# rrahn/libspm

Measured on AMD Instinct MI355X. Metric: Gbases/s scanned, Myers k<=3 |P|=100, higher is better.
Workload: dtype u32

## Files before the change

libspm_amd/csrc/filter.hpp:

```cpp
#pragma once

#include "brute.hpp"
#include "common.hpp"
#include "filter_shared.hpp"
#include "pack.hpp"
#include "hd.hpp"

namespace spm_hip
{

struct survivor
{
    uint32_t key;
    uint32_t t_lo, t_hi;
    uint32_t pad;
};
constexpr uint32_t kSurvInvalid = 0xFFFFFFFFu;

struct band_rec
{
    uint32_t slot;
    uint32_t val;
    uint32_t seg;
    uint32_t band;
// ... 295 lines not shown
            const bool act = todo != 0;
            const uint32_t b = act ? (uint32_t)__ffs(todo) - 1u : 0u;
            todo &= todo - 1;
            const uint32_t u = b & 1u, d = (b >> 1) + 1u;
            const uint32_t wu = (j + 1 < NWD && u) ? w[j + 1 < NWD ? j + 1 : j] : w[j];
            const uint32_t pu = (j + 1 < NWD && u) ? prev[j + 1 < NWD ? j + 1 : j] : prev[j];
            const uint32_t key = (uint32_t)((((uint64_t)wu << 32) | pu) >> (2 * d));
            const uint32_t x = chd_hash(key).x;
            const uint32_t dsp = disp_tab[x >> P.chd_bucket_shift];
            const uint32_t slot = ((x >> 3) + dsp * ((key | 1u) & 0xFFFFFFu)) & P.chd_slot_mask;
            const uint32_t f = fp_tab[slot];
            const bool hit = act && ((f ^ key ^ (key >> 16)) & 0xFFFFu) == 0;
            if (__ballot(hit) != 0) {
                if (__builtin_amdgcn_readfirstlane(cand_chunk_of(P, lds)[5]) != 0)
                    return;
                const uint64_t wpos = gbase + (uint64_t)(j + u) * 1024 + (uint64_t)lane * 16;
                const int64_t ts = (int64_t)wpos - 16 + (int64_t)d;
                const bool has = hit && ts >= (int64_t)P.lo && (uint64_t)ts + P.key_len <= P.hi;
                emit_survivors(P, has, key, has ? (uint64_t)ts : 0, lane, lds);
            }
        }
    }
}

template <int S, int UU, int HV, int SIG, bool KM, bool AN = false>
__device__ __forceinline__ void filter_group(const filter_params &P, const uint4 (&cur)[UU], uint64_t gbase,
                                             uint32_t &carry_in, uint32_t &carry_n, uint32_t lane,
                                             const uint32_t *lds, uint32_t idx_mask)
{
    uint32_t w[UU], prev[UU];
    uint32_t nv[SIG != 4 ? UU : 1];
#pragma unroll
    for (int u = 0; u < UU; ++u) {
        uint32_t nm = 0;
        w[u] = pack16_sig<SIG>(cur[u], nm);
        prev[u] = __builtin_amdgcn_update_dpp(0u, w[u], 0x138 , 0xF, 0xF, false);
        if (lane == 0)
            prev[u] = carry_in;
        carry_in = __builtin_amdgcn_readlane(w[u], 63);
        if (SIG != 4) {
            uint32_t np = __builtin_amdgcn_update_dpp(0u, nm, 0x138, 0xF, 0xF, false);
            if (lane == 0)
                np = carry_n;
            carry_n = __builtin_amdgcn_readlane(nm, 63);
            nv[u] = (nm << 16) | np;
        }
    }
    if constexpr (AN)
        filter_words_anchored<UU>(P, w, prev, gbase, lane, lds);
    else
        filter_words<S, UU, HV, SIG, false, KM>(P, w, prev, nv, gbase, lane, lds, idx_mask);
}

template <int S, int U, int HV, int SIG, bool KM, bool AN = false>
__global__ __launch_bounds__(((S == 1 && !KM && SIG == 4) || (S == 2 && U == 2)) ? 1024 : 512) void seed_filter_kernel(const filter_params P)
{
    extern __shared__ uint32_t lds[];
    for (uint32_t i = threadIdx.x; i < P.lds_words; i += blockDim.x)
        lds[i] = P.bitmap[i];
    if ((threadIdx.x & 63) == 0) {
        uint32_t *ck = lds + P.lds_words + kCandLdsSlot + kCandRec * (threadIdx.x >> 6);
        for (uint32_t i = 0; i < kCandRec; ++i)
            ck[i] = 0;
    }
    __syncthreads();

    const uint32_t lane = threadIdx.x & 63;
    const uint32_t waves_per_wg = blockDim.x >> 6;
    const uint64_t wave_id =
        (uint64_t)blockIdx.x * waves_per_wg + (uint32_t)__builtin_amdgcn_readfirstlane(threadIdx.x >> 6);
    const uint64_t n_waves = (uint64_t)gridDim.x * waves_per_wg;
    const uint32_t idx_mask = P.bitmap_words * 32 - 1;

    const uint64_t base0 = P.lo & ~1023ull;
    const uint64_t n_chunks = (P.hi - base0 + 1023) / 1024;
    const uint64_t n_whole = (P.hi - base0) / 1024;
    const uint64_t span = P.span_chunks;
    const uint64_t n_spans = (n_chunks + span - 1) / span;
    const uint8_t *lane_text = P.text + base0 + (uint64_t)lane * 16;

    const uint32_t wave_in_wg = (uint32_t)__builtin_amdgcn_readfirstlane(threadIdx.x >> 6);
    uint64_t sp = wave_id;
    for (;;) {
        if (P.dynamic == 1) {
            unsigned long long t = 0;
            if (lane == 0)
                t = atomicAdd(&P.counters[kCntSpanHead], 1ull);
            sp = ((unsigned long long)__builtin_amdgcn_readfirstlane((uint32_t)(t >> 32)) << 32) |
                 (uint32_t)__builtin_amdgcn_readfirstlane((uint32_t)t);
        } else if (P.dynamic == 2) {
            __syncthreads();
            if (threadIdx.x == 0) {
                const unsigned long long t = atomicAdd(&P.counters[kCntSpanHead], (unsigned long long)waves_per_wg);
                lds[P.lds_words] = (uint32_t)t;
                lds[P.lds_words + 1] = (uint32_t)(t >> 32);
            }
            __syncthreads();
            const uint64_t base = ((uint64_t)(uint32_t)__builtin_amdgcn_readfirstlane(lds[P.lds_words + 1]) << 32) |
                                  (uint32_t)__builtin_amdgcn_readfirstlane(lds[P.lds_words]);
            if (base >= n_spans)
                break;
            sp = base + wave_in_wg;
            if (sp >= n_spans)
                continue;
        }
        if (sp >= n_spans)
            break;
        const uint64_t c_begin = sp * span;
        const uint64_t c_end = c_begin + span < n_chunks ? c_begin + span : n_chunks;
        span_open(P, lds, lane, base0 + c_begin * 1024);
        uint32_t carry_in = 0, carry_n = 0;
        {
            const uint64_t cb = base0 + c_begin * 1024;
            if (cb >= 16 && lane == 0) {
                const uint4 before = load_text16(P.text, cb - 16, P.hi);
                carry_in = pack16_sig<SIG>(before, carry_n);
            }
            carry_in = __builtin_amdgcn_readfirstlane(carry_in);
            carry_n = __builtin_amdgcn_readfirstlane(carry_n);
        }
        uint64_t ch = c_begin;
        const uint64_t whole_end = c_end < n_whole ? c_end : n_whole;
        const uint64_t fast_end = c_begin + (whole_end > c_begin ? (whole_end - c_begin) / U * U : 0);
        if (ch < fast_end) {
            uint4 nxt[U];
#pragma unroll
            for (int u = 0; u < U; ++u)
                nxt[u] = load16_stream(lane_text + (ch + u) * 1024);
            for (; ch < fast_end; ch += U) {
                uint4 cur[U];
#pragma unroll
                for (int u = 0; u < U; ++u)
                    cur[u] = nxt[u];
                const bool more = ch + U < fast_end;
                const uint64_t pf = more ? ch + U : ch;
                const uint64_t ustride = more ? 1024 : 0;
#pragma unroll
                for (int u = 0; u < U; ++u)
                    nxt[u] = load16_stream(lane_text + pf * 1024 + (uint64_t)u * ustride);
                if constexpr (S <= 2)
                    __builtin_amdgcn_sched_barrier(0);
                filter_group<S, U, HV, SIG, KM, AN>(P, cur, base0 + ch * 1024, carry_in, carry_n, lane, lds, idx_mask);
            }
        }
        for (; ch < c_end; ++ch) {
            uint4 one[1];
            one[0] = load_text16(P.text, base0 + ch * 1024 + (uint64_t)lane * 16, P.hi);
            filter_group<S, 1, HV, SIG, KM, AN>(P, one, base0 + ch * 1024, carry_in, carry_n, lane, lds, idx_mask);
        }
        sp += n_waves;
    }
    surv_close(P, cand_chunk_of(P, lds), lane);
}

constexpr uint32_t kDenseQueueCap = 192;
constexpr int kDenseBatches = 3;

template <int NP>
__device__ __forceinline__ uint32_t dense_select(const filter_params &P, uint32_t w, uint32_t prev)
{
    const uint32_t X = alignbit(w, prev, 2);
    const uint32_t Y = alignbit(w, prev, 4);
    uint32_t sel = 0;
#pragma unroll
    for (int i = 0; i < NP; ++i) {
        const uint32_t C0 = (P.pat_c[i] & 3u) * 0x55555555u, M0 = (P.pat_cm[i] & 3u) * 0x55555555u;
        const uint32_t C1 = (P.pat_c[i] >> 2) * 0x55555555u, M1 = (P.pat_cm[i] >> 2) * 0x55555555u;
        uint32_t t = ((X ^ C0) & M0) | ((Y ^ C1) & M1);
        t |= t >> 1;
        sel |= ~t;
    }
    return sel & 0x55555555u;
}

struct dense_queue
{
    uint32_t key[kDenseQueueCap];
    uint32_t off[kDenseQueueCap];
};

__device__ __forceinline__ void dense_drain(const filter_params &P, dense_queue &Q, uint32_t &qn, bool all, uint64_t span_base,
                                            uint32_t lane, const uint32_t *lds)
{
    while (qn >= 64 || (all && qn != 0)) {
        const uint32_t nb_full = qn >> 6;
        uint32_t nb = all ? (qn + 63) >> 6 : nb_full;
        nb = nb > (uint32_t)kDenseBatches ? (uint32_t)kDenseBatches : nb;
        uint32_t key[kDenseBatches], off[kDenseBatches];
        uint4 bk[kDenseBatches];
        bool v[kDenseBatches];
#pragma unroll
        for (int b = 0; b < kDenseBatches; ++b) {
            const int32_t e = (int32_t)qn - 64 * b - 1 - (int32_t)lane;
            v[b] = (uint32_t)b < nb && e >= 0;
            key[b] = 0;
            off[b] = 0;
            bk[b] = make_uint4(0, 0, 0, 0);
            if (v[b]) {
                key[b] = Q.key[e];
                off[b] = Q.off[e];
                bk[b] = P.buckets[dense_bucket(key[b], P.bucket_shift)];
            }
        }
// ... 42 lines not shown
        uint32_t pm = 0;
        if constexpr (S == 0) {
            uint32_t todo = dense_select<NP>(P, w0, p0);
            if (pair)
                todo |= dense_select<NP>(P, w1, p1) << 1;
            while (todo != 0) {
                const uint32_t b = (uint32_t)__ffs(todo) - 1u;
                todo &= todo - 1;
                const bool odd = (b & 1u) != 0;
                const uint64_t both = ((uint64_t)(odd ? w1 : w0) << 32) | (odd ? p1 : p0);
                const uint32_t key = (uint32_t)(both >> ((b & ~1u) + 2u));
                const uint32_t h = key ^ (key >> 13);
                const uint32_t word = *reinterpret_cast<const uint32_t *>(reinterpret_cast<const uint8_t *>(lds) + ((h >> 3) & 0x1FFFCu));
                pm |= __builtin_amdgcn_ubfe(word, h, 1) << b;
            }
        } else {
#pragma unroll
            for (int u = 0; u < (pair ? 2 : 1); ++u) {
#pragma unroll
                for (int d = S; d <= 16; d += S) {
                    const uint32_t wu = u ? w1 : w0, pu = u ? p1 : p0;
                    const uint32_t key = (d == 16 ? wu : alignbit(wu, pu, (2 * d) & 31)) & kmask;
                    const uint32_t h = key ^ (key >> 13);
                    const uint32_t word = *reinterpret_cast<const uint32_t *>(reinterpret_cast<const uint8_t *>(lds) + ((h >> 3) & 0x1FFFCu));
                    pm |= __builtin_amdgcn_ubfe(word, h, 1) << (2 * (d - 1) + u);
                }
            }
        }
        while (__ballot(pm != 0) != 0) {
            const bool pos = pm != 0;
            const uint32_t b = pos ? (uint32_t)__ffs(pm) - 1u : 0u;
            pm &= pm - 1;
            const bool odd = (b & 1u) != 0;
            const uint64_t both = ((uint64_t)(odd ? w1 : w0) << 32) | (odd ? p1 : p0);
            const uint32_t key = (uint32_t)(both >> ((b & ~1u) + 2u)) & kmask;
            const uint64_t mm = __ballot(pos);
            if (pos) {
                const uint32_t q = qn + __popcll(mm & ((1ull << lane) - 1));
                Q.key[q] = key;
                Q.off[q] = goff + (uint32_t)j * 1024u + (odd ? 1024u : 0u) + (b >> 1) + 1u;
            }
            qn += __popcll(mm);
            __builtin_amdgcn_fence(__ATOMIC_RELEASE, "wavefront");
            __builtin_amdgcn_wave_barrier();
            if (qn > kDenseQueueCap - 64)
                dense_drain(P, Q, qn, false, span_base, lane, lds);
        }
    }
}

template <int U, int NP, int S = 0, bool KM = false>
__global__ __launch_bounds__(1024) void seed_filter_dense_kernel(const filter_params P)
{
    extern __shared__ uint32_t lds[];
    for (uint32_t i = threadIdx.x; i < P.lds_words; i += blockDim.x)
        lds[i] = P.bitmap[i];
    if ((threadIdx.x & 63) == 0) {
        uint32_t *ck = lds + P.lds_words + kCandLdsSlot + kCandRec * (threadIdx.x >> 6);
        for (uint32_t i = 0; i < kCandRec; ++i)
            ck[i] = 0;
    }
    __syncthreads();

    const uint32_t lane = threadIdx.x & 63;
    const uint32_t waves_per_wg = blockDim.x >> 6;
    const uint32_t wave_in_wg = (uint32_t)__builtin_amdgcn_readfirstlane(threadIdx.x >> 6);
    const uint64_t wave_id = (uint64_t)blockIdx.x * waves_per_wg + wave_in_wg;
    const uint64_t n_waves = (uint64_t)gridDim.x * waves_per_wg;
    dense_queue &Q = *reinterpret_cast<dense_queue *>(lds + P.lds_words + kCandLdsSlot + kCandRec * 16 +
                                                      (sizeof(dense_queue) / 4) * wave_in_wg);
    uint32_t qn = 0;

    const uint64_t base0 = P.lo & ~1023ull;
    const uint64_t n_chunks = (P.hi - base0 + 1023) / 1024;
    const uint64_t n_whole = (P.hi - base0) / 1024;
    const uint64_t span = P.span_chunks;
    const uint64_t n_spans = (n_chunks + span - 1) / span;
    const uint8_t *lane_text = P.text + base0 + (uint64_t)lane * 16;

    uint64_t sp = wave_id;
    for (;;) {
        if (P.dynamic == 1) {
            unsigned long long t = 0;
            if (lane == 0)
                t = atomicAdd(&P.counters[kCntSpanHead], 1ull);
            sp = ((unsigned long long)__builtin_amdgcn_readfirstlane((uint32_t)(t >> 32)) << 32) |
                 (uint32_t)__builtin_amdgcn_readfirstlane((uint32_t)t);
        } else if (P.dynamic == 2) {
            __syncthreads();
            if (threadIdx.x == 0) {
                const unsigned long long t = atomicAdd(&P.counters[kCntSpanHead], (unsigned long long)waves_per_wg);
                lds[P.lds_words] = (uint32_t)t;
                lds[P.lds_words + 1] = (uint32_t)(t >> 32);
            }
            __syncthreads();
            const uint64_t base = ((uint64_t)(uint32_t)__builtin_amdgcn_readfirstlane(lds[P.lds_words + 1]) << 32) |
                                  (uint32_t)__builtin_amdgcn_readfirstlane(lds[P.lds_words]);
            if (base >= n_spans)
                break;
            sp = base + wave_in_wg;
            if (sp >= n_spans)
                continue;
        }
        if (sp >= n_spans)
            break;
        const uint64_t c_begin = sp * span;
        const uint64_t c_end = c_begin + span < n_chunks ? c_begin + span : n_chunks;
        const uint64_t span_base = base0 + c_begin * 1024;
        span_open(P, lds, lane, span_base);
        uint32_t carry_in = 0;
        {
            uint32_t nm = 0;
            if (span_base >= 16 && lane == 0)
                carry_in = pack16_sig<4>(load_text16(P.text, span_base - 16, P.hi), nm);
            carry_in = __builtin_amdgcn_readfirstlane(carry_in);
        }
        uint64_t ch = c_begin;
        const uint64_t whole_end = c_end < n_whole ? c_end : n_whole;
        const uint64_t fast_end = c_begin + (whole_end > c_begin ? (whole_end - c_begin) / U * U : 0);
        if (ch < fast_end) {
            uint4 nxt[U];
#pragma unroll
            for (int u = 0; u < U; ++u)
                nxt[u] = load16_stream(lane_text + (ch + u) * 1024);
            for (; ch < fast_end; ch += U) {
                uint4 cur[U];
#pragma unroll
                for (int u = 0; u < U; ++u)
                    cur[u] = nxt[u];
                const bool more = ch + U < fast_end;
                const uint64_t pf = more ? ch + U : ch;
                const uint64_t ustride = more ? 1024 : 0;
#pragma unroll
                for (int u = 0; u < U; ++u)
                    nxt[u] = load16_stream(lane_text + pf * 1024 + (uint64_t)u * ustride);
                __builtin_amdgcn_sched_barrier(0);
                dense_group<U, NP, S, KM>(P, cur, base0 + ch * 1024, span_base, carry_in, lane, lds, Q, qn);
            }
        }
        for (; ch < c_end; ++ch) {
            uint4 one[1];
            one[0] = load_text16(P.text, base0 + ch * 1024 + (uint64_t)lane * 16, P.hi);
            dense_group<1, NP, S, KM>(P, one, base0 + ch * 1024, span_base, carry_in, lane, lds, Q, qn);
        }
        dense_drain(P, Q, qn, true, span_base, lane, lds);
        sp += n_waves;
    }
    surv_close(P, cand_chunk_of(P, lds), lane);
}

template <int S, int U2, int HV, bool KM>
__global__ __launch_bounds__(1024) void seed_filter_packed_kernel(const filter_params P, const uint4 *__restrict__ shadow)
{
    extern __shared__ uint32_t lds[];
    for (uint32_t i = threadIdx.x; i < P.lds_words; i += blockDim.x)
        lds[i] = P.bitmap[i];
    if ((threadIdx.x & 63) == 0) {
        uint32_t *ck = lds + P.lds_words + kCandLdsSlot + kCandRec * (threadIdx.x >> 6);
        for (uint32_t i = 0; i < kCandRec; ++i)
            ck[i] = 0;
    }
    __syncthreads();

    constexpr int NWD = 4 * U2;
    const uint32_t lane = threadIdx.x & 63;
    const uint32_t waves_per_wg = blockDim.x >> 6;
    const uint32_t wave_in_wg = (uint32_t)__builtin_amdgcn_readfirstlane(threadIdx.x >> 6);
    const uint64_t wave_id = (uint64_t)blockIdx.x * waves_per_wg + wave_in_wg;
    const uint64_t n_waves = (uint64_t)gridDim.x * waves_per_wg;
    const uint32_t idx_mask = P.bitmap_words * 32 - 1;

    const uint64_t base0 = P.lo & ~4095ull;
    const uint64_t n_chunks = (P.hi - base0 + 4095) / 4096;
    const uint64_t span = P.span_chunks;
    const uint64_t n_spans = (n_chunks + span - 1) / span;
    const uint4 *lane_src = shadow + (base0 / 64) + lane;

    uint64_t sp = wave_id;
    for (;;) {
        if (P.dynamic == 1) {
            unsigned long long t = 0;
            if (lane == 0)
                t = atomicAdd(&P.counters[kCntSpanHead], 1ull);
            sp = ((unsigned long long)__builtin_amdgcn_readfirstlane((uint32_t)(t >> 32)) << 32) |
                 (uint32_t)__builtin_amdgcn_readfirstlane((uint32_t)t);
        } else if (P.dynamic == 2) {
            __syncthreads();
            if (threadIdx.x == 0) {
                const unsigned long long t = atomicAdd(&P.counters[kCntSpanHead], (unsigned long long)waves_per_wg);
                lds[P.lds_words] = (uint32_t)t;
                lds[P.lds_words + 1] = (uint32_t)(t >> 32);
            }
            __syncthreads();
            const uint64_t base = ((uint64_t)(uint32_t)__builtin_amdgcn_readfirstlane(lds[P.lds_words + 1]) << 32) |
                                  (uint32_t)__builtin_amdgcn_readfirstlane(lds[P.lds_words]);
            if (base >= n_spans)
                break;
            sp = base + wave_in_wg;
            if (sp >= n_spans)
                continue;
        }
        if (sp >= n_spans)
            break;
        const uint64_t c_begin = sp * span;
        const uint64_t c_end = c_begin + span < n_chunks ? c_begin + span : n_chunks;
        const uint64_t fast_end = c_begin + (c_end - c_begin + U2 - 1) / U2 * U2;
        span_open(P, lds, lane, base0 + c_begin * 4096);
        uint32_t carry_in = 0;
        {
            const uint64_t first_word = (base0 + c_begin * 4096) / 16;
            if (first_word > 0 && lane == 0)
                carry_in = reinterpret_cast<const uint32_t *>(shadow)[first_word - 1];
            carry_in = __builtin_amdgcn_readfirstlane(carry_in);
        }
        uint4 nxt[U2];
#pragma unroll
        for (int u = 0; u < U2; ++u)
            nxt[u] = load16_stream(reinterpret_cast<const uint8_t *>(lane_src + (c_begin + u) * 64));
        for (uint64_t ch = c_begin; ch < fast_end; ch += U2) {
            uint4 cur[U2];
#pragma unroll
            for (int u = 0; u < U2; ++u)
                cur[u] = nxt[u];
            const bool more = ch + U2 < fast_end;
            const uint64_t pf = more ? ch + U2 : ch;
            const uint64_t ustride = more ? 64 : 0;
#pragma unroll
            for (int u = 0; u < U2; ++u)
                nxt[u] = load16_stream(reinterpret_cast<const uint8_t *>(lane_src + pf * 64 + (uint64_t)u * ustride));
            __builtin_amdgcn_sched_barrier(0);
            uint32_t w[NWD], prev[NWD];
            const uint32_t nv[1] = {0};
#pragma unroll
            for (int u = 0; u < U2; ++u) {
                w[4 * u + 0] = cur[u].x;
                w[4 * u + 1] = cur[u].y;
                w[4 * u + 2] = cur[u].z;
                w[4 * u + 3] = cur[u].w;
                uint32_t p0 = __builtin_amdgcn_update_dpp(0u, cur[u].w, 0x138 , 0xF, 0xF, false);
                if (lane == 0)
                    p0 = carry_in;
                carry_in = __builtin_amdgcn_readlane(cur[u].w, 63);
                prev[4 * u + 0] = p0;
                prev[4 * u + 1] = cur[u].x;
                prev[4 * u + 2] = cur[u].y;
                prev[4 * u + 3] = cur[u].z;
            }
            filter_words<S, NWD, HV, 4, true, KM>(P, w, prev, nv, base0 + ch * 4096, lane, lds, idx_mask);
        }
        sp += n_waves;
    }
    surv_close(P, cand_chunk_of(P, lds), lane);
}

struct verify_params
{
    const uint8_t *text;
    uint64_t text_alloc;
    uint64_t ctx_begin;
    uint64_t scan_begin;
    uint64_t scan_end;
    uint64_t pos_offset;
    const band_rec *bands;
    const unsigned long long *counters;
    uint32_t band_counter;
    uint32_t preselected;
    uint64_t band_cap;
    ulonglong2 *band_tab;
    uint32_t table_mask, band_bits;
    uint32_t runs;
    const uint8_t *surplus;
    uint32_t Bw;
    uint32_t overlap;
    uint32_t max_m;
    const uint32_t *peq32;
    uint32_t sigma;
    uint32_t nw_table;
    uint32_t max_k;
    const int32_t *m;
    const int32_t *k;
    uint32_t report_begin;
    uint32_t max_span;
    uint32_t wave_text;
    unsigned long long *seen;
    uint32_t seen_mask;
    spm_hit *hits;
    unsigned long long *hit_counter;
    uint64_t hit_cap;
    unsigned long long *overflow;
    const uint64_t *seg_offsets;
    uint64_t n_segments;
    const uint32_t *seg_owned;
};

struct resolve_params
{
    const survivor *surv;
    unsigned long long *counters;
    uint64_t surv_cap;
    const pass_entry *passes;
    const uint4 *entries;
    uint32_t key_len;
    uint32_t flank_check;
// ... 1254 lines not shown
```

libspm_amd/csrc/internal.hpp:

```cpp
#pragma once

#include <algorithm>
#include <chrono>
#include <cmath>
#include <cstdlib>
#include <cstring>
#include <memory>

#include "common.hpp"
#include "index_build.hpp"

using namespace spm_hip;

struct spm_patterns : spm_hip::seed_index
{
    spm_ctx *ctx = nullptr;
    int algo = 0;
    uint32_t n = 0;
    uint32_t sigma = 4;
    std::vector<uint8_t> ranks;
    std::vector<uint32_t> offsets;
    std::vector<int32_t> m, k;
    uint32_t n_groups = 0;
    uint32_t max_m = 0;
    uint32_t max_window = 0;
    uint32_t max_k = 0;
    uint32_t NW = 1;
    bool is_myers() const { return algo == SPM_ALGO_MYERS || algo == SPM_ALGO_MYERS_PREFIX; }
    void *d_arena = nullptr;
    uint32_t *d_peq = nullptr;
    uint32_t *d_peq_bot = nullptr;
    uint32_t *d_peq_verify = nullptr;
    uint32_t *d_hp0 = nullptr;
    int32_t *d_m = nullptr;
    int32_t *d_k = nullptr;
    mutable uint64_t cand_hint = 0;
    uint8_t *d_surplus = nullptr;
    uint8_t *d_ranks = nullptr;
    uint32_t *d_offsets = nullptr;
    uint32_t *d_needle_pk = nullptr;
    uint32_t *d_pk_offsets = nullptr;
    uint16_t *d_seed_q = nullptr;
    pass_entry *d_pass_tab = nullptr;
    uint4 *d_entries = nullptr;
    mutable uint64_t hit_hint = 0;
    mutable bool scanned = false;
    mutable int exact_whole = -1;
    mutable uint64_t band_hint = 0;
    spm_build_stats build{};
    mutable void *d_align = nullptr;
    mutable const uint64_t *d_al_rpeq = nullptr;
    mutable const uint32_t *d_al_rpeq_off = nullptr;
    mutable const uint8_t *d_al_ranks = nullptr;
    mutable const uint32_t *d_al_offsets = nullptr;
};

using clk = std::chrono::steady_clock;
inline float ms_since(clk::time_point t) { return std::chrono::duration<float, std::milli>(clk::now() - t).count(); }
inline bool spm_trace_on()
{
    const char *v = getenv("SPM_HIP_TRACE");
    return v && *v && *v != '0';
}


struct scan_tuning
{
    int cand_cap = 0;
    int brute_cutoff = 1;
    int verify_wave_min_words = 8;
    int span_budget = 0;
    int verify_runs = 1;
    int verify_runs_min_bands = 65536;
    int band_cap = 0;
    static scan_tuning from_env()
    {
        scan_tuning T;
        T.cand_cap = env_int("SPM_HIP_FILTER_CAND_CAP", 0);
        T.brute_cutoff = env_int("SPM_HIP_BRUTE_CUTOFF", 1);
        T.verify_wave_min_words = env_int("SPM_HIP_VERIFY_WAVE_MIN_WORDS", 8);
        T.span_budget = env_int("SPM_HIP_FILTER_SPAN_BUDGET", 0);
        T.verify_runs = env_int("SPM_HIP_VERIFY_RUNS", 1);
        T.verify_runs_min_bands = env_int("SPM_HIP_VERIFY_RUNS_MIN_BANDS", 65536);
        T.band_cap = env_int("SPM_HIP_FILTER_BAND_CAP", 0);
        return T;
    }
};

struct scan_args
{
    spm_ctx *ctx;
    const spm_text *text;
    uint64_t begin, end, ctx_begin;
    const spm_patterns *ps;
    spm_scan_opts opts;
    spm_hits *hits;
    scan_tuning tune;
    const uint64_t *seg_offsets = nullptr;
    uint64_t n_segments = 0;
    const uint64_t *d_seg_offsets = nullptr;
    const uint32_t *d_seg_owned = nullptr;
};

struct scan_state
{
    retry_state retry;
    filter_result filt;
    const uint64_t *segs = nullptr;
    std::vector<uint64_t> seg_host;
    const std::vector<uint64_t> *tiles = nullptr;
};

void state_to_internal(const spm_patterns *p, const void *state, std::vector<uint32_t> &out);
void state_from_internal(const spm_patterns *p, const std::vector<uint32_t> &in, void *state);
int text_alloc(spm_ctx *ctx, uint64_t n, uint32_t sigma, spm_text **out);
int ensure_scratch(spm_ctx *ctx, size_t bytes);
int run_brute(const scan_args &A, const scan_state &S, uint64_t begin, uint64_t end, uint64_t ctx_begin,
              const uint32_t *d_state_in, uint32_t *d_state_out, bool report, bool single_tile);
int run_filter(const scan_args &A, const retry_state &R, filter_result &out);
int scan_impl(spm_ctx *ctx, const spm_text *text, uint64_t begin, uint64_t end, const spm_patterns *patterns,
              const spm_scan_opts *opts_in, const void *state_in, void *state_out, const uint64_t *seg_offsets,
              uint64_t n_segments, spm_hits **out, const uint64_t *d_seg_offsets = nullptr,
              const uint32_t *d_seg_owned = nullptr, const std::function<int(spm_hits *)> *after_launch = nullptr);

struct align_work
{
    const spm_patterns *ps = nullptr;
    const spm_text *text = nullptr;
    uint64_t pos_offset = 0;
    const spm_hit *hits = nullptr;
    uint64_t n = 0;
    const uint64_t *lo = nullptr;
    const uint32_t *cig_off = nullptr;
    bool begin_only = false;
// ... 18 lines not shown
```

libspm_amd/csrc/scan_filter.hip:

```cpp
#include "internal.hpp"
#include "filter.hpp"

namespace
{
template <typename K, typename... Args>
void launch(K kernel, dim3 grid, uint32_t threads, size_t lds, hipStream_t s, Args... args)
{
    hipFuncSetAttribute((const void *)kernel, hipFuncAttributeMaxDynamicSharedMemorySize, (int)lds);
    hipLaunchKernelGGL(kernel, grid, dim3(threads), lds, s, args...);
}

using filter_kernel = void (*)(filter_params);
using packed_kernel = void (*)(filter_params, const uint4 *);

template <int S, int U, bool KM>
filter_kernel sparse_kernel(uint32_t hv, uint32_t sigma)
{
    if (hv == 2 && sigma == 5)
        return seed_filter_kernel<S, U, 2, 5, KM>;
    if (hv == 2 && sigma == 15)
        return seed_filter_kernel<S, U, 2, 15, KM>;
    if (hv == 1 && sigma == 4)
        return seed_filter_kernel<S, U, 1, 4, KM>;
    if constexpr (S >= 4)
// ... 19 lines not shown
        if (F.stride == 2)
            return km ? seed_filter_dense_kernel<4, 1, 2, true> : seed_filter_dense_kernel<4, 1, 2, false>;
        return nullptr;
    }
    switch (F.stride) {
    case 16: return km ? nullptr : sparse_kernel<16, 8, false>(F.hash_variant, sigma);
    case 8: return km ? nullptr : sparse_kernel<8, 8, false>(F.hash_variant, sigma);
    case 4: return km ? nullptr : sparse_kernel<4, 8, false>(F.hash_variant, sigma);
    case 2: return km ? sparse_kernel<2, 2, true>(F.hash_variant, sigma) : sparse_kernel<2, 2, false>(F.hash_variant, sigma);
    case 1:
        if (F.anchor_cm != 0 && F.hash_variant == 2 && sigma == 4 && !km)
            return seed_filter_kernel<1, 4, 2, 4, false, true>;
        return km ? sparse_kernel<1, 2, true>(F.hash_variant, sigma) : sparse_kernel<1, 2, false>(F.hash_variant, sigma);
    default: return nullptr;
    }
}

packed_kernel select_packed_kernel(uint32_t stride, bool km)
{
    if (km)
        return nullptr;
    switch (stride) {
    case 16: return seed_filter_packed_kernel<16, 4, 2, false>;
    case 8: return seed_filter_packed_kernel<8, 4, 2, false>;
    case 4: return seed_filter_packed_kernel<4, 2, 2, false>;
    default: return nullptr;
    }
}

template <int NWN>
void launch_verify_nw(const verify_params &V, dim3 grid, hipStream_t s)
{
    uint32_t threads = 256;
    const size_t per_thread = (size_t)(V.sigma + 1) * NWN * 4 + 2 * 16;
    while (threads > 64 && per_thread * threads > 128 * 1024)
        threads >>= 1;
    const size_t lds = per_thread * threads + (size_t)(threads / 64) * kHitStage * sizeof(spm_hit);
    launch(verify_kernel<NWN>, grid, threads, lds, s, V);
}

template <int G>
void launch_verify_wave_g(verify_params V, const uint32_t *peq_bot, uint32_t max_m, dim3 grid, hipStream_t s)
{
    grid.x *= 4;
    const uint32_t n_slots = 2 * V.max_k + 1 + V.max_span;
    V.wave_text = ((max_m + V.max_k + n_slots + 16 + 15) & ~15u) + 16;
    const size_t per_group = ((n_slots * 2 + 15) & ~15u) + V.wave_text;
    launch(verify_wave_kernel<G, 1>, grid, 64, (64 / G) * per_group, s, V, peq_bot);
}

void launch_verify_wave(uint32_t n_blocks, const verify_params &V, const uint32_t *peq_bot, uint32_t max_m, dim3 grid,
                        hipStream_t s)
{
    if (n_blocks <= 8)
        launch_verify_wave_g<8>(V, peq_bot, max_m, grid, s);
    else if (n_blocks <= 16)
        launch_verify_wave_g<16>(V, peq_bot, max_m, grid, s);
    else if (n_blocks <= 32)
        launch_verify_wave_g<32>(V, peq_bot, max_m, grid, s);
    else
        launch_verify_wave_g<64>(V, peq_bot, max_m, grid, s);
}

void launch_verify(uint32_t nwn, const verify_params &V, dim3 grid, hipStream_t s)
{
    switch (nwn) {
    case 1: launch_verify_nw<1>(V, grid, s); break;
    case 2: launch_verify_nw<2>(V, grid, s); break;
    case 3: launch_verify_nw<3>(V, grid, s); break;
    case 4: launch_verify_nw<4>(V, grid, s); break;
    case 5: launch_verify_nw<5>(V, grid, s); break;
    case 6: launch_verify_nw<6>(V, grid, s); break;
    case 7: launch_verify_nw<7>(V, grid, s); break;
    case 8: launch_verify_nw<8>(V, grid, s); break;
    case 16: launch_verify_nw<16>(V, grid, s); break;
    case 32: launch_verify_nw<32>(V, grid, s); break;
    default: launch_verify_nw<64>(V, grid, s); break;
    }
}

}

int ensure_band_table(spm_ctx *ctx, uint64_t slots)
{
    if (ctx->band_slots >= slots && !ctx->band_dirty)
        return SPM_OK;
    if (ctx->band_slots < slots) {
        const auto t0 = clk::now();
        if (ctx->d_band_tab) {
            SPM_HIP_CHECK(ctx, hipStreamSynchronize(ctx->stream));
            hipFree(ctx->d_band_tab);
            ctx->d_band_tab = nullptr;
            ctx->band_slots = 0;
        }
        SPM_HIP_CHECK(ctx, hipMalloc(&ctx->d_band_tab, slots * sizeof(ulonglong2)));
        ctx->band_slots = slots;
        if (spm_trace_on())
            fprintf(stderr, "[spm_hip] band table grows to %.1f MiB: %.2f ms\n", slots * sizeof(ulonglong2) / 1048576.0, ms_since(t0));
    }
    SPM_HIP_CHECK(ctx, hipMemsetAsync(ctx->d_band_tab, 0xFF, ctx->band_slots * sizeof(ulonglong2), ctx->stream));
    SPM_HIP_CHECK(ctx, hipMemsetAsync(ctx->d_table_poison, 0, 4, ctx->stream));
    ctx->band_dirty = false;
    return SPM_OK;
}

namespace
{
// ... 44 lines not shown
    int launch_passes()
    {
        filter_params P{};
        P.text = A.text->d;
        P.text_alloc = A.text->owned ? A.text->alloc : A.text->n;
        const uint64_t reach = ps->max_window;
        P.lo = A.begin >= A.ctx_begin + reach ? A.begin - reach : A.ctx_begin;
        P.hi = A.end;
        P.surv = surv;
        P.counters = H->d_count;
        P.surv_cap = Z.surv_cap;
        P.ovf_spans = ovf;
        P.ovf_cap = kOvfCap;
        for (size_t fi = 0; fi < ps->fidx.size(); ++fi) {
            const filter_index &F = ps->fidx[fi];
            P.stride = F.stride;
            P.key_len = F.key_len;
            P.key_mask = F.key_len >= 16 ? 0xFFFFFFFFu : ((1u << (2 * F.key_len)) - 1);
            P.bitmap_words = F.hash_variant == 2 ? 1024 : F.bitmap_words;
            P.lds_words = F.lds_words;
            P.chd_slot_mask = F.chd_slot_mask;
            P.chd_bucket_shift = F.chd_bucket_shift;
            P.chd_disp_off = F.chd_disp_off;
            P.n_probes = F.n_probes;
            P.bitmap = F.d_bitmap;
            P.pass = (uint32_t)fi;
            P.anchor_c = F.anchor_c;
            P.anchor_cm = F.anchor_cm;
            P.n_pat = F.n_pat;
            for (uint32_t i = 0; i < kDensePatterns; ++i) {
                P.pat_c[i] = F.pat_c[i];
                P.pat_cm[i] = F.pat_cm[i];
            }
            P.bucket_shift = F.bucket_shift;
            P.buckets = reinterpret_cast<const uint4 *>(F.d_buckets);
            if (fi > 0)
                SPM_HIP_CHECK(ctx, hipMemsetAsync(H->d_count + kCntSpanHead, 0, sizeof(unsigned long long), ctx->stream));
            const bool km = F.key_len < 16;
            const bool bits = F.hash_variant == 4;
            const bool use_packed = F.hash_variant == 2 && A.text->d_packed && ps->sigma == 4 && F.stride >= 2 &&
                                    !(A.opts.flags & SPM_SCAN_IGNORE_PACKED);
            const bool wide_ok = use_packed || F.stride == 2 || (F.stride == 1 && !km && ps->sigma == 4);
            const uint32_t threads = (F.dense || bits || wide_ok) ? 1024 : 512;
            const size_t lds = (size_t)F.lds_words * 4 + 16 + 16 * kCandRec * 4 + ((F.dense || bits) ? 16 * sizeof(dense_queue) : 0);
            const uint32_t wg_per_cu = (uint32_t)std::max<size_t>(1, std::min<size_t>((160 * 1024) / lds, 2048 / threads));
            const uint32_t grid = ctx->n_cu * wg_per_cu;
            const uint64_t n_waves = (uint64_t)grid * (threads / 64);
            const uint64_t n_chunks = (P.hi - (P.lo & ~1023ull) + 1023) / 1024;
            const span_plan span = plan_span(n_chunks, n_waves, 1024);
            P.span_chunks = span.span_chunks;
            P.span_unit = 1024;
            const int sb = A.tune.span_budget;
            P.span_budget = sb > 0 ? (uint32_t)sb : (uint32_t)std::max<uint64_t>(256, (uint64_t)span.span_chunks * 1024 / 4);
            P.dynamic = span.dynamic;
            P.hash_variant = F.hash_variant;
            H->stats.span_symbols = P.span_chunks * P.span_unit;
            if (use_packed) {
                filter_params Q = P;
                const uint64_t n_pchunks = (Q.hi - (Q.lo & ~4095ull) + 4095) / 4096;
                const span_plan pspan = plan_span(n_pchunks, n_waves, 4096);
                Q.span_chunks = pspan.span_chunks;
                Q.span_unit = 4096;
                if (sb <= 0)
                    Q.span_budget = (uint32_t)std::max<uint64_t>(256, (uint64_t)pspan.span_chunks * 4096 / 4);
                Q.dynamic = pspan.dynamic;
                H->stats.span_symbols = Q.span_chunks * Q.span_unit;
                const packed_kernel k = select_packed_kernel(F.stride, km);
                if (!k) {
                    SPM_SET_ERR(ctx, "internal: no packed filter kernel for stride %u, key length %u", F.stride, F.key_len);
                    return SPM_E_UNSUPPORTED;
                }
                launch(k, dim3(grid), threads, lds, ctx->stream, Q, reinterpret_cast<const uint4 *>(A.text->d_packed));
            } else {
                const filter_kernel k = select_filter_kernel(F, ps->sigma, km);
                if (!k) {
                    SPM_SET_ERR(ctx, "internal: no filter kernel for stride %u, key length %u, sigma %u, hash variant %u, %u patterns",
                                F.stride, F.key_len, ps->sigma, F.hash_variant, F.n_pat);
                    return SPM_E_UNSUPPORTED;
                }
                launch(k, dim3(grid), threads, lds, ctx->stream, P);
            }
            SPM_HIP_CHECK(ctx, hipGetLastError());
            H->stats.main_launches++;
        }
        return SPM_OK;
    }

    template <typename Params>
    void fill_shared(Params &X) const
    {
        X.text = A.text->d;
        X.text_alloc = A.text->owned ? A.text->alloc : A.text->n;
        X.scan_begin = A.begin;
        X.scan_end = A.end;
        X.pos_offset = A.opts.pos_offset;
        X.counters = H->d_count;
        X.bands = bands;
        X.band_cap = Z.band_cap;
        X.band_tab = ctx->d_band_tab;
        X.table_mask = (uint32_t)(Z.band_slots - 1);
        X.band_bits = 43 - seg_bits;
        X.Bw = Z.Bw;
        X.overlap = Z.overlap ? 1u : 0u;
        X.max_m = ps->max_m;
        X.m = ps->d_m;
        X.k = ps->d_k;
        X.report_begin = ps->is_myers() ? 0 : 1;
        X.seen_mask = (uint32_t)(Z.seen_slots - 1);
        X.hits = H->d_hits;
        X.hit_counter = H->d_count + kCntHits;
        X.overflow = H->d_count + kCntVoid;
        X.hit_cap = H->cap;
        X.seg_offsets = d_seg;
        X.n_segments = n_seg;
        X.seg_owned = A.d_seg_owned;
    }

    int launch_resolve()
    {
        if (A.d_seg_offsets) {
            d_seg = A.d_seg_offsets;
            n_seg = A.n_segments;
        } else if (A.seg_offsets) {
            uint64_t *d = nullptr;
            SPM_HIP_CHECK(ctx, hipMalloc(&d, (A.n_segments + 1) * sizeof(uint64_t)));
            hipFree(H->d_aux[1]);
            H->d_aux[1] = d;
            SPM_HIP_CHECK(ctx, hipMemcpyAsync(d, A.seg_offsets, (A.n_segments + 1) * sizeof(uint64_t),
                                              hipMemcpyHostToDevice, ctx->stream));
            d_seg = d;
            n_seg = A.n_segments;
        }
        while (n_seg && (1ull << seg_bits) < n_seg + 1)
            ++seg_bits;
        resolve_params R{};
        fill_shared(R);
        R.surv = surv;
        R.surv_cap = Z.surv_cap;
        R.passes = ps->d_pass_tab;
        R.entries = ps->d_entries;
        R.key_len = ps->filter_key_len;
        R.needle_ranks = ps->d_ranks;
        R.needle_offsets = ps->d_offsets;
        R.seed_q = ps->d_seed_q;
        R.flank_check = (ps->sigma == 4 && !Z.overlap && R.needle_ranks) ? 1u : 0u;
        R.pieces_check = R.flank_check;
        R.hay_begin = A.ctx_begin;
        R.hay_end = A.end;
        R.needle_pk = ps->d_needle_pk;
        R.pk_offsets = ps->d_pk_offsets;
        R.exact_hits = exact_hits ? 1u : 0u;
        R.seen = skip_seen ? nullptr : seen;
        R.table_poison = ctx->d_table_poison;
        const uint64_t surv_expect = ps->cand_hint ? 2 * ps->cand_hint : Z.surv_cap;
        const uint64_t rmax = (uint64_t)ctx->n_cu * 5;
        const uint64_t per_wg = (surv_expect + 255) / 256 <= rmax ? 256 : 1024;
        const uint32_t rgrid = (uint32_t)std::min<uint64_t>(rmax, std::max<uint64_t>(ctx->n_cu / 2, (surv_expect + per_wg - 1) / per_wg));
        hipLaunchKernelGGL(resolve_kernel, dim3(rgrid), dim3(256), 0, ctx->stream, R);
        SPM_HIP_CHECK(ctx, hipGetLastError());
        return SPM_OK;
    }

    int launch_bands(bool runs)
    {
        verify_params V{};
        fill_shared(V);
        V.ctx_begin = A.ctx_begin;
        V.surplus = ps->d_surplus;
        V.peq32 = ps->d_peq_verify ? ps->d_peq_verify : ps->d_peq;
        V.sigma = ps->sigma;
        V.nw_table = ps->NW;
        V.max_k = ps->max_k;
        V.max_span = Z.max_span;
        V.seen = seen;
        V.band_counter = kCntBandSlots;
        band_rec *kept = bands + Z.band_cap;
        if (runs) {
            hipLaunchKernelGGL(band_runs_kernel, dim3(ctx->n_cu * 8), dim3(256), 0, ctx->stream, V, bands, kept, H->d_count + kCntRunHeads);
            SPM_HIP_CHECK(ctx, hipGetLastError());
            V.runs = 1;
            V.bands = kept;
            V.band_counter = kCntRunHeads;
        }
        if (Z.overlap) {
            hipLaunchKernelGGL(band_select_kernel, dim3(ctx->n_cu * 2), dim3(256), 0, ctx->stream, V, kept, H->d_count + kCntBandsSelected);
            SPM_HIP_CHECK(ctx, hipGetLastError());
            V.bands = kept;
            V.band_counter = kCntBandsSelected;
            V.preselected = 1;
        }
        if (exact_hits) {
        } else if (Z.use_wave) {
            launch_verify_wave(Z.nwn, V, ps->d_peq_bot, ps->max_m, dim3(ctx->n_cu * 16), ctx->stream);
        } else {
            const uint32_t nwn = Z.nwn > 8 ? ps->NW : Z.nwn;
            const uint64_t band_expect = ps->band_hint ? 2 * ps->band_hint : Z.band_cap;
            const uint32_t vgrid = (uint32_t)std::min<uint64_t>((uint64_t)ctx->n_cu * 4, std::max<uint64_t>(ctx->n_cu / 2, (band_expect + 255) / 256));
            launch_verify(nwn, V, dim3(vgrid), ctx->stream);
        }
        SPM_HIP_CHECK(ctx, hipGetLastError());
        if (runs) {
            hipLaunchKernelGGL(band_release_kernel, dim3(ctx->n_cu * 8), dim3(256), 0, ctx->stream, V, bands, (uint32_t)kCntBandSlots);
            SPM_HIP_CHECK(ctx, hipGetLastError());
        }
        return SPM_OK;
    }
};

}

int run_filter(const scan_args &A, const retry_state &R, filter_result &out)
{
    spm_ctx *ctx = A.ctx;
    spm_hits *H = A.hits;
    filter_run F{A, R, ctx, A.ps, H, size_filter(*A.ps, A.tune, A.end - A.begin, (uint64_t)ctx->n_cu, H->cap, R)};
    const filter_sizes &Z = F.Z;
    SPM_TRY(F.lay_out());
    const bool runs = !Z.overlap && !F.exact_hits && !Z.use_wave && Z.Bw <= 32 && !R.need_seen && A.tune.verify_runs != 0 &&
                      A.ps->band_hint >= (uint64_t)std::max(0, A.tune.verify_runs_min_bands);
    out = {F.seen, (uint32_t)(Z.seen_slots - 1), F.ovf, F.skip_seen || runs, Z.surv_cap, Z.band_cap};
    SPM_HIP_CHECK(ctx, hipEventRecord(H->ev[1], ctx->stream));
    SPM_TRY(F.launch_passes());
    SPM_HIP_CHECK(ctx, hipEventRecord(H->ev[2], ctx->stream));
    SPM_TRY(F.launch_resolve());
    SPM_TRY(F.launch_bands(runs));
    SPM_HIP_CHECK(ctx, hipEventRecord(H->ev[3], ctx->stream));
    return SPM_OK;
}


void spm_warm_filter_kernels()
{
    hipFuncAttributes a;
    (void)hipFuncGetAttributes(&a, (const void *)resolve_kernel);
}
```

Before: 6504.

## Overlap first span text loads with LDS image staging and add narrow wave verify

Issues each wave's first span text loads and boundary carry load before the bitmap image is copied into LDS. This hides global-memory latency behind the staging copy, which now uses batched 16-byte vector loads. The span-dequeue logic moves into a shared helper, with the first span assigned statically and an env override for the dequeue mode. Wave-level verify gains 2- and 4-word instantiations and is chosen for small band counts, which adds template variants and more heuristic branches.

```diff
diff --git a/libspm_amd/csrc/filter.hpp b/libspm_amd/csrc/filter.hpp
--- a/libspm_amd/csrc/filter.hpp
+++ b/libspm_amd/csrc/filter.hpp
@@ -371,23 +371,86 @@
         filter_words<S, UU, HV, SIG, false, KM>(P, w, prev, nv, gbase, lane, lds, idx_mask);
 }
 
+
+constexpr int kStageBatch = 8;
+
+__device__ __forceinline__ void stage_image(const filter_params &P, uint32_t *lds)
+{
+    const uint32_t n = P.lds_words;
+    const uint32_t n4 = (reinterpret_cast<uintptr_t>(P.bitmap) & 15u) == 0 ? n >> 2 : 0u;
+    if (n4 != 0) {
+        const uint4 *src = reinterpret_cast<const uint4 *>(P.bitmap);
+        uint4 *dst = reinterpret_cast<uint4 *>(lds);
+        for (uint32_t b = threadIdx.x; b < n4; b += kStageBatch * blockDim.x) {
+            uint4 v[kStageBatch];
+#pragma unroll
+            for (int j = 0; j < kStageBatch; ++j) {
+                const uint32_t i = b + (uint32_t)j * blockDim.x;
+                v[j] = src[i < n4 ? i : n4 - 1];
+            }
+#pragma unroll
+            for (int j = 0; j < kStageBatch; ++j) {
+                const uint32_t i = b + (uint32_t)j * blockDim.x;
+                dst[i < n4 ? i : n4 - 1] = v[j];
+            }
+        }
+    }
+    for (uint32_t i = 4 * n4 + threadIdx.x; i < n; i += blockDim.x)
+        lds[i] = P.bitmap[i];
+    if ((threadIdx.x & 63) == 0) {
+        uint32_t *ck = lds + n + kCandLdsSlot + kCandRec * (threadIdx.x >> 6);
+        for (uint32_t i = 0; i < kCandRec; ++i)
+            ck[i] = 0;
+    }
+    __syncthreads();
+}
+
+enum span_turn { kSpanLeave, kSpanScan, kSpanIdle };
+
+__device__ __forceinline__ span_turn next_span(const filter_params &P, uint32_t *lds, bool first, uint64_t n_waves,
+                                               uint64_t n_spans, uint32_t wave_in_wg, uint32_t lane, uint64_t &sp)
+{
+    const uint32_t waves_per_wg = blockDim.x >> 6;
+    if (P.dynamic == 2) {
+        uint64_t base = (uint64_t)blockIdx.x * waves_per_wg;
+        if (!first) {
+            __syncthreads();
+            if (threadIdx.x == 0) {
+                const unsigned long long t = atomicAdd(&P.counters[kCntSpanHead], (unsigned long long)waves_per_wg);
+                lds[P.lds_words] = (uint32_t)t;
+                lds[P.lds_words + 1] = (uint32_t)(t >> 32);
+            }
+            __syncthreads();
+            base = n_waves + (((uint64_t)(uint32_t)__builtin_amdgcn_readfirstlane(lds[P.lds_words + 1]) << 32) |
+                              (uint32_t)__builtin_amdgcn_readfirstlane(lds[P.lds_words]));
+        }
+        if (base >= n_spans)
+            return kSpanLeave;
+        sp = base + wave_in_wg;
+        return sp < n_spans ? kSpanScan : kSpanIdle;
+    }
+    if (!first) {
+        if (P.dynamic == 1) {
+            unsigned long long t = 0;
+            if (lane == 0)
+                t = atomicAdd(&P.counters[kCntSpanHead], 1ull);
+            sp = n_waves + (((unsigned long long)__builtin_amdgcn_readfirstlane((uint32_t)(t >> 32)) << 32) |
+                            (uint32_t)__builtin_amdgcn_readfirstlane((uint32_t)t));
+        } else {
+            sp += n_waves;
+        }
+    }
+    return sp < n_spans ? kSpanScan : kSpanLeave;
+}
+
 template <int S, int U, int HV, int SIG, bool KM, bool AN = false>
 __global__ __launch_bounds__(((S == 1 && !KM && SIG == 4) || (S == 2 && U == 2)) ? 1024 : 512) void seed_filter_kernel(const filter_params P)
 {
-    extern __shared__ uint32_t lds[];
-    for (uint32_t i = threadIdx.x; i < P.lds_words; i += blockDim.x)
-        lds[i] = P.bitmap[i];
-    if ((threadIdx.x & 63) == 0) {
-        uint32_t *ck = lds + P.lds_words + kCandLdsSlot + kCandRec * (threadIdx.x >> 6);
-        for (uint32_t i = 0; i < kCandRec; ++i)
-            ck[i] = 0;
-    }
-    __syncthreads();
-
+    extern __shared__ __align__(16) uint32_t lds[];
     const uint32_t lane = threadIdx.x & 63;
     const uint32_t waves_per_wg = blockDim.x >> 6;
-    const uint64_t wave_id =
-        (uint64_t)blockIdx.x * waves_per_wg + (uint32_t)__builtin_amdgcn_readfirstlane(threadIdx.x >> 6);
+    const uint32_t wave_in_wg = (uint32_t)__builtin_amdgcn_readfirstlane(threadIdx.x >> 6);
+    const uint64_t wave_id = (uint64_t)blockIdx.x * waves_per_wg + wave_in_wg;
     const uint64_t n_waves = (uint64_t)gridDim.x * waves_per_wg;
     const uint32_t idx_mask = P.bitmap_words * 32 - 1;
 
@@ -398,43 +461,47 @@
     const uint64_t n_spans = (n_chunks + span - 1) / span;
     const uint8_t *lane_text = P.text + base0 + (uint64_t)lane * 16;
 
-    const uint32_t wave_in_wg = (uint32_t)__builtin_amdgcn_readfirstlane(threadIdx.x >> 6);
+    uint4 nxt[U], before;
+    auto span_first_loads = [&](uint64_t s) {
+        const uint64_t c_begin = s * span;
+        const uint64_t c_end = c_begin + span < n_chunks ? c_begin + span : n_chunks;
+        const uint64_t whole_end = c_end < n_whole ? c_end : n_whole;
+        const uint64_t cb = base0 + c_begin * 1024;
+        before = make_uint4(0, 0, 0, 0);
+        if (cb >= 16 && lane == 0)
+            before = load_text16(P.text, cb - 16, P.hi);
+        if (whole_end >= c_begin + U) {
+#pragma unroll
+            for (int u = 0; u < U; ++u)
+                nxt[u] = load16_stream(lane_text + (c_begin + u) * 1024);
+        }
+    };
     uint64_t sp = wave_id;
-    for (;;) {
-        if (P.dynamic == 1) {
-            unsigned long long t = 0;
-            if (lane == 0)
-                t = atomicAdd(&P.counters[kCntSpanHead], 1ull);
-            sp = ((unsigned long long)__builtin_amdgcn_readfirstlane((uint32_t)(t >> 32)) << 32) |
-                 (uint32_t)__builtin_amdgcn_readfirstlane((uint32_t)t);
-        } else if (P.dynamic == 2) {
-            __syncthreads();
-            if (threadIdx.x == 0) {
-                const unsigned long long t = atomicAdd(&P.counters[kCntSpanHead], (unsigned long long)waves_per_wg);
-                lds[P.lds_words] = (uint32_t)t;
-                lds[P.lds_words + 1] = (uint32_t)(t >> 32);
-            }
-            __syncthreads();
-            const uint64_t base = ((uint64_t)(uint32_t)__builtin_amdgcn_readfirstlane(lds[P.lds_words + 1]) << 32) |
-                                  (uint32_t)__builtin_amdgcn_readfirstlane(lds[P.lds_words]);
-            if (base >= n_spans)
-                break;
-            sp = base + wave_in_wg;
-            if (sp >= n_spans)
-                continue;
-        }
-        if (sp >= n_spans)
+    bool loaded = sp < n_spans;
+#pragma unroll
+    for (int u = 0; u < U; ++u)
+        nxt[u] = make_uint4(0, 0, 0, 0);
+    before = make_uint4(0, 0, 0, 0);
+    if (loaded)
+        span_first_loads(sp);
+    __builtin_amdgcn_sched_barrier(0);
+    stage_image(P, lds);
+
+    for (bool first = true;; first = false) {
+        const span_turn turn = next_span(P, lds, first, n_waves, n_spans, wave_in_wg, lane, sp);
+        if (turn == kSpanLeave)
             break;
+        if (turn == kSpanIdle)
+            continue;
         const uint64_t c_begin = sp * span;
         const uint64_t c_end = c_begin + span < n_chunks ? c_begin + span : n_chunks;
+        if (!loaded)
+            span_first_loads(sp);
+        loaded = false;
         span_open(P, lds, lane, base0 + c_begin * 1024);
         uint32_t carry_in = 0, carry_n = 0;
-        {
-            const uint64_t cb = base0 + c_begin * 1024;
-            if (cb >= 16 && lane == 0) {
-                const uint4 before = load_text16(P.text, cb - 16, P.hi);
-                carry_in = pack16_sig<SIG>(before, carry_n);
-            }
+        if (base0 + c_begin * 1024 >= 16) {
+            carry_in = pack16_sig<SIG>(before, carry_n);
             carry_in = __builtin_amdgcn_readfirstlane(carry_in);
             carry_n = __builtin_amdgcn_readfirstlane(carry_n);
         }
@@ -442,10 +509,6 @@
         const uint64_t whole_end = c_end < n_whole ? c_end : n_whole;
         const uint64_t fast_end = c_begin + (whole_end > c_begin ? (whole_end - c_begin) / U * U : 0);
         if (ch < fast_end) {
-            uint4 nxt[U];
-#pragma unroll
-            for (int u = 0; u < U; ++u)
-                nxt[u] = load16_stream(lane_text + (ch + u) * 1024);
             for (; ch < fast_end; ch += U) {
                 uint4 cur[U];
 #pragma unroll
@@ -467,7 +530,6 @@
             one[0] = load_text16(P.text, base0 + ch * 1024 + (uint64_t)lane * 16, P.hi);
             filter_group<S, 1, HV, SIG, KM, AN>(P, one, base0 + ch * 1024, carry_in, carry_n, lane, lds, idx_mask);
         }
-        sp += n_waves;
     }
     surv_close(P, cand_chunk_of(P, lds), lane);
 }
@@ -616,16 +678,7 @@
 template <int U, int NP, int S = 0, bool KM = false>
 __global__ __launch_bounds__(1024) void seed_filter_dense_kernel(const filter_params P)
 {
-    extern __shared__ uint32_t lds[];
-    for (uint32_t i = threadIdx.x; i < P.lds_words; i += blockDim.x)
-        lds[i] = P.bitmap[i];
-    if ((threadIdx.x & 63) == 0) {
-        uint32_t *ck = lds + P.lds_words + kCandLdsSlot + kCandRec * (threadIdx.x >> 6);
-        for (uint32_t i = 0; i < kCandRec; ++i)
-            ck[i] = 0;
-    }
-    __syncthreads();
-
+    extern __shared__ __align__(16) uint32_t lds[];
     const uint32_t lane = threadIdx.x & 63;
     const uint32_t waves_per_wg = blockDim.x >> 6;
     const uint32_t wave_in_wg = (uint32_t)__builtin_amdgcn_readfirstlane(threadIdx.x >> 6);
@@ -642,51 +695,54 @@
     const uint64_t n_spans = (n_chunks + span - 1) / span;
     const uint8_t *lane_text = P.text + base0 + (uint64_t)lane * 16;
 
+    uint4 nxt[U], before;
+    auto span_first_loads = [&](uint64_t s) {
+        const uint64_t c_begin = s * span;
+        const uint64_t c_end = c_begin + span < n_chunks ? c_begin + span : n_chunks;
+        const uint64_t whole_end = c_end < n_whole ? c_end : n_whole;
+        const uint64_t cb = base0 + c_begin * 1024;
+        before = make_uint4(0, 0, 0, 0);
+        if (cb >= 16 && lane == 0)
+            before = load_text16(P.text, cb - 16, P.hi);
+        if (whole_end >= c_begin + U) {
+#pragma unroll
+            for (int u = 0; u < U; ++u)
+                nxt[u] = load16_stream(lane_text + (c_begin + u) * 1024);
+        }
+    };
     uint64_t sp = wave_id;
-    for (;;) {
-        if (P.dynamic == 1) {
-            unsigned long long t = 0;
-            if (lane == 0)
-                t = atomicAdd(&P.counters[kCntSpanHead], 1ull);
-            sp = ((unsigned long long)__builtin_amdgcn_readfirstlane((uint32_t)(t >> 32)) << 32) |
-                 (uint32_t)__builtin_amdgcn_readfirstlane((uint32_t)t);
-        } else if (P.dynamic == 2) {
-            __syncthreads();
-            if (threadIdx.x == 0) {
-                const unsigned long long t = atomicAdd(&P.counters[kCntSpanHead], (unsigned long long)waves_per_wg);
-                lds[P.lds_words] = (uint32_t)t;
-                lds[P.lds_words + 1] = (uint32_t)(t >> 32);
-            }
-            __syncthreads();
-            const uint64_t base = ((uint64_t)(uint32_t)__builtin_amdgcn_readfirstlane(lds[P.lds_words + 1]) << 32) |
-                                  (uint32_t)__builtin_amdgcn_readfirstlane(lds[P.lds_words]);
-            if (base >= n_spans)
-                break;
-            sp = base + wave_in_wg;
-            if (sp >= n_spans)
-                continue;
-        }
-        if (sp >= n_spans)
+    bool loaded = sp < n_spans;
+#pragma unroll
+    for (int u = 0; u < U; ++u)
+        nxt[u] = make_uint4(0, 0, 0, 0);
+    before = make_uint4(0, 0, 0, 0);
+    if (loaded)
+        span_first_loads(sp);
+    __builtin_amdgcn_sched_barrier(0);
+    stage_image(P, lds);
+
+    for (bool first = true;; first = false) {
+        const span_turn turn = next_span(P, lds, first, n_waves, n_spans, wave_in_wg, lane, sp);
+        if (turn == kSpanLeave)
             break;
+        if (turn == kSpanIdle)
+            continue;
         const uint64_t c_begin = sp * span;
         const uint64_t c_end = c_begin + span < n_chunks ? c_begin + span : n_chunks;
         const uint64_t span_base = base0 + c_begin * 1024;
+        if (!loaded)
+            span_first_loads(sp);
+        loaded = false;
         span_open(P, lds, lane, span_base);
         uint32_t carry_in = 0;
-        {
+        if (span_base >= 16) {
             uint32_t nm = 0;
-            if (span_base >= 16 && lane == 0)
-                carry_in = pack16_sig<4>(load_text16(P.text, span_base - 16, P.hi), nm);
-            carry_in = __builtin_amdgcn_readfirstlane(carry_in);
+            carry_in = __builtin_amdgcn_readfirstlane(pack16_sig<4>(before, nm));
         }
         uint64_t ch = c_begin;
         const uint64_t whole_end = c_end < n_whole ? c_end : n_whole;
         const uint64_t fast_end = c_begin + (whole_end > c_begin ? (whole_end - c_begin) / U * U : 0);
         if (ch < fast_end) {
-            uint4 nxt[U];
-#pragma unroll
-            for (int u = 0; u < U; ++u)
-                nxt[u] = load16_stream(lane_text + (ch + u) * 1024);
             for (; ch < fast_end; ch += U) {
                 uint4 cur[U];
 #pragma unroll
@@ -708,7 +764,6 @@
             dense_group<1, NP, S, KM>(P, one, base0 + ch * 1024, span_base, carry_in, lane, lds, Q, qn);
         }
         dense_drain(P, Q, qn, true, span_base, lane, lds);
-        sp += n_waves;
     }
     surv_close(P, cand_chunk_of(P, lds), lane);
 }
@@ -716,16 +771,7 @@
 template <int S, int U2, int HV, bool KM>
 __global__ __launch_bounds__(1024) void seed_filter_packed_kernel(const filter_params P, const uint4 *__restrict__ shadow)
 {
-    extern __shared__ uint32_t lds[];
-    for (uint32_t i = threadIdx.x; i < P.lds_words; i += blockDim.x)
-        lds[i] = P.bitmap[i];
-    if ((threadIdx.x & 63) == 0) {
-        uint32_t *ck = lds + P.lds_words + kCandLdsSlot + kCandRec * (threadIdx.x >> 6);
-        for (uint32_t i = 0; i < kCandRec; ++i)
-            ck[i] = 0;
-    }
-    __syncthreads();
-
+    extern __shared__ __align__(16) uint32_t lds[];
     constexpr int NWD = 4 * U2;
     const uint32_t lane = threadIdx.x & 63;
     const uint32_t waves_per_wg = blockDim.x >> 6;
@@ -740,47 +786,42 @@
     const uint64_t n_spans = (n_chunks + span - 1) / span;
     const uint4 *lane_src = shadow + (base0 / 64) + lane;
 
+    uint4 nxt[U2];
+    uint32_t before = 0;
+    auto span_first_loads = [&](uint64_t s) {
+        const uint64_t c_begin = s * span;
+        const uint64_t first_word = (base0 + c_begin * 4096) / 16;
+        before = 0;
+        if (first_word > 0 && lane == 0)
+            before = reinterpret_cast<const uint32_t *>(shadow)[first_word - 1];
+#pragma unroll
+        for (int u = 0; u < U2; ++u)
+            nxt[u] = load16_stream(reinterpret_cast<const uint8_t *>(lane_src + (c_begin + u) * 64));
+    };
     uint64_t sp = wave_id;
-    for (;;) {
-        if (P.dynamic == 1) {
-            unsigned long long t = 0;
-            if (lane == 0)
-                t = atomicAdd(&P.counters[kCntSpanHead], 1ull);
-            sp = ((unsigned long long)__builtin_amdgcn_readfirstlane((uint32_t)(t >> 32)) << 32) |
-                 (uint32_t)__builtin_amdgcn_readfirstlane((uint32_t)t);
-        } else if (P.dynamic == 2) {
-            __syncthreads();
-            if (threadIdx.x == 0) {
-                const unsigned long long t = atomicAdd(&P.counters[kCntSpanHead], (unsigned long long)waves_per_wg);
-                lds[P.lds_words] = (uint32_t)t;
-                lds[P.lds_words + 1] = (uint32_t)(t >> 32);
-            }
-            __syncthreads();
-            const uint64_t base = ((uint64_t)(uint32_t)__builtin_amdgcn_readfirstlane(lds[P.lds_words + 1]) << 32) |
-                                  (uint32_t)__builtin_amdgcn_readfirstlane(lds[P.lds_words]);
-            if (base >= n_spans)
-                break;
-            sp = base + wave_in_wg;
-            if (sp >= n_spans)
-                continue;
-        }
-        if (sp >= n_spans)
+    bool loaded = sp < n_spans;
+#pragma unroll
+    for (int u = 0; u < U2; ++u)
+        nxt[u] = make_uint4(0, 0, 0, 0);
+    if (loaded)
+        span_first_loads(sp);
+    __builtin_amdgcn_sched_barrier(0);
+    stage_image(P, lds);
+
+    for (bool first = true;; first = false) {
+        const span_turn turn = next_span(P, lds, first, n_waves, n_spans, wave_in_wg, lane, sp);
+        if (turn == kSpanLeave)
             break;
+        if (turn == kSpanIdle)
+            continue;
         const uint64_t c_begin = sp * span;
         const uint64_t c_end = c_begin + span < n_chunks ? c_begin + span : n_chunks;
         const uint64_t fast_end = c_begin + (c_end - c_begin + U2 - 1) / U2 * U2;
+        if (!loaded)
+            span_first_loads(sp);
+        loaded = false;
         span_open(P, lds, lane, base0 + c_begin * 4096);
-        uint32_t carry_in = 0;
-        {
-            const uint64_t first_word = (base0 + c_begin * 4096) / 16;
-            if (first_word > 0 && lane == 0)
-                carry_in = reinterpret_cast<const uint32_t *>(shadow)[first_word - 1];
-            carry_in = __builtin_amdgcn_readfirstlane(carry_in);
-        }
-        uint4 nxt[U2];
-#pragma unroll
-        for (int u = 0; u < U2; ++u)
-            nxt[u] = load16_stream(reinterpret_cast<const uint8_t *>(lane_src + (c_begin + u) * 64));
+        uint32_t carry_in = __builtin_amdgcn_readfirstlane(before);
         for (uint64_t ch = c_begin; ch < fast_end; ch += U2) {
             uint4 cur[U2];
 #pragma unroll
@@ -812,7 +853,6 @@
             }
             filter_words<S, NWD, HV, 4, true, KM>(P, w, prev, nv, base0 + ch * 4096, lane, lds, idx_mask);
         }
-        sp += n_waves;
     }
     surv_close(P, cand_chunk_of(P, lds), lane);
 }
diff --git a/libspm_amd/csrc/internal.hpp b/libspm_amd/csrc/internal.hpp
--- a/libspm_amd/csrc/internal.hpp
+++ b/libspm_amd/csrc/internal.hpp
@@ -64,12 +64,15 @@
 }
 
 
+constexpr int kVerifyWaveMinWordsDefault = 8;
+
 struct scan_tuning
 {
     int cand_cap = 0;
     int brute_cutoff = 1;
-    int verify_wave_min_words = 8;
+    int verify_wave_min_words = kVerifyWaveMinWordsDefault;
     int span_budget = 0;
+    int span_dequeue = 0;
     int verify_runs = 1;
     int verify_runs_min_bands = 65536;
     int band_cap = 0;
@@ -78,8 +81,9 @@
         scan_tuning T;
         T.cand_cap = env_int("SPM_HIP_FILTER_CAND_CAP", 0);
         T.brute_cutoff = env_int("SPM_HIP_BRUTE_CUTOFF", 1);
-        T.verify_wave_min_words = env_int("SPM_HIP_VERIFY_WAVE_MIN_WORDS", 8);
+        T.verify_wave_min_words = env_int("SPM_HIP_VERIFY_WAVE_MIN_WORDS", kVerifyWaveMinWordsDefault);
         T.span_budget = env_int("SPM_HIP_FILTER_SPAN_BUDGET", 0);
+        T.span_dequeue = env_int("SPM_HIP_FILTER_SPAN_DEQUEUE", 0);
         T.verify_runs = env_int("SPM_HIP_VERIFY_RUNS", 1);
         T.verify_runs_min_bands = env_int("SPM_HIP_VERIFY_RUNS_MIN_BANDS", 65536);
         T.band_cap = env_int("SPM_HIP_FILTER_BAND_CAP", 0);
diff --git a/libspm_amd/csrc/scan_filter.hip b/libspm_amd/csrc/scan_filter.hip
--- a/libspm_amd/csrc/scan_filter.hip
+++ b/libspm_amd/csrc/scan_filter.hip
@@ -95,7 +95,11 @@
 void launch_verify_wave(uint32_t n_blocks, const verify_params &V, const uint32_t *peq_bot, uint32_t max_m, dim3 grid,
                         hipStream_t s)
 {
-    if (n_blocks <= 8)
+    if (n_blocks <= 2)
+        launch_verify_wave_g<2>(V, peq_bot, max_m, grid, s);
+    else if (n_blocks <= 4)
+        launch_verify_wave_g<4>(V, peq_bot, max_m, grid, s);
+    else if (n_blocks <= 8)
         launch_verify_wave_g<8>(V, peq_bot, max_m, grid, s);
     else if (n_blocks <= 16)
         launch_verify_wave_g<16>(V, peq_bot, max_m, grid, s);
@@ -246,7 +250,8 @@
             P.span_unit = 1024;
             const int sb = A.tune.span_budget;
             P.span_budget = sb > 0 ? (uint32_t)sb : (uint32_t)std::max<uint64_t>(256, (uint64_t)span.span_chunks * 1024 / 4);
-            P.dynamic = span.dynamic;
+            const uint32_t dq = (A.tune.span_dequeue == 1 || A.tune.span_dequeue == 2) ? (uint32_t)A.tune.span_dequeue : 0u;
+            P.dynamic = dq ? dq : span.dynamic;
             P.hash_variant = F.hash_variant;
             H->stats.span_symbols = P.span_chunks * P.span_unit;
             if (use_packed) {
@@ -257,7 +262,7 @@
                 Q.span_unit = 4096;
                 if (sb <= 0)
                     Q.span_budget = (uint32_t)std::max<uint64_t>(256, (uint64_t)pspan.span_chunks * 4096 / 4);
-                Q.dynamic = pspan.dynamic;
+                Q.dynamic = dq ? dq : pspan.dynamic;
                 H->stats.span_symbols = Q.span_chunks * Q.span_unit;
                 const packed_kernel k = select_packed_kernel(F.stride, km);
                 if (!k) {
@@ -355,6 +360,16 @@
         return SPM_OK;
     }
 
+    bool narrow_wave(bool runs) const
+    {
+        if (A.tune.verify_wave_min_words != kVerifyWaveMinWordsDefault)
+            return false;
+        if (Z.overlap || runs || ps->sigma > 5 || !ps->d_peq_bot || Z.nwn < 2 || Z.nwn > 7 || ps->band_hint == 0)
+            return false;
+        const uint64_t G = Z.nwn <= 2 ? 2 : Z.nwn <= 4 ? 4 : 8;
+        return 2 * ps->band_hint * G <= (uint64_t)ctx->n_cu * 4 * 64;
+    }
+
     int launch_bands(bool runs)
     {
         verify_params V{};
@@ -384,7 +399,7 @@
             V.preselected = 1;
         }
         if (exact_hits) {
-        } else if (Z.use_wave) {
+        } else if (Z.use_wave || narrow_wave(runs)) {
             launch_verify_wave(Z.nwn, V, ps->d_peq_bot, ps->max_m, dim3(ctx->n_cu * 16), ctx->stream);
         } else {
             const uint32_t nwn = Z.nwn > 8 ? ps->NW : Z.nwn;
```

After: 6614 (median of 6 runs). 1.7% higher.
